# diegoroyo/mitransient

Measured on AMD Instinct MI355X. Metric: Mray/s (closest-hit + shadow rays), Cornell-box 512^2 x 1024 bins x 1024 spp per GPU, higher is better.
Workload: dtype f32; 1 GPU; cornell_box() diffuse, 512x512 px, 1024 time bins (start_opl 3.5, width 6/1024), 1024 spp per GPU (1024 spp total), max_depth 8, rr_depth 5, seed 0; parallelism=1 GPU, mode=auto (fused: scene + per-pixel time histograms in LDS)

## Files before the change

### mitransient_amd/csrc/mtr_core.h

```cpp
#pragma once
#ifndef MTR_WIDE
#define MTR_WIDE 8
#endif

#include <stdint.h>
#include <math.h>
#include "../../include/mitransient_amd.h"

#if defined(__HIPCC__)
#include <hip/hip_runtime.h>
#define MTR_HD __host__ __device__ __forceinline__
#else
#define MTR_HD inline __attribute__((always_inline))
#endif

namespace mtr {

struct f3 { float x, y, z; };

MTR_HD f3 mk(float x, float y, float z) { f3 r; r.x = x; r.y = y; r.z = z; return r; }
MTR_HD f3 operator-(f3 a, f3 b) { return mk(a.x - b.x, a.y - b.y, a.z - b.z); }
MTR_HD f3 operator-(f3 a) { return mk(-a.x, -a.y, -a.z); }
MTR_HD f3 operator*(f3 a, float s) { return mk(a.x * s, a.y * s, a.z * s); }
MTR_HD f3 operator/(f3 a, float s) { float r = 1.0f / s; return mk(a.x * r, a.y * r, a.z * r); }
MTR_HD float dot(f3 a, f3 b) { return fmaf(a.x, b.x, fmaf(a.y, b.y, a.z * b.z)); }
MTR_HD f3 cross(f3 a, f3 b)
{
    return mk(fmaf(a.y, b.z, -(a.z * b.y)), fmaf(a.z, b.x, -(a.x * b.z)), fmaf(a.x, b.y, -(a.y * b.x)));
}
MTR_HD f3 normalize(f3 a) { return a / sqrtf(dot(a, a)); }
MTR_HD f3 fma3(f3 a, float s, f3 b) { return mk(fmaf(a.x, s, b.x), fmaf(a.y, s, b.y), fmaf(a.z, s, b.z)); }
MTR_HD float max3(float a, float b, float c) { return fmaxf(a, fmaxf(b, c)); }
MTR_HD bool sign_neg(float s) { return s < 0.0f || (s == 0.0f && signbit(s)); }

constexpr float kPi = 3.14159265358979323846f;
constexpr float kInvPi = 0.31830988618379067154f;
constexpr float kRayEps = 1500.0f * 5.9604644775390625e-8f;
constexpr float kShadowEps = kRayEps * 10.0f;
constexpr float kInf = __builtin_huge_valf();
constexpr float kEdgeEps = 1.9073486328125e-06f;
// ... 425 lines not shown
        const q4 X = n.q[0], Y = n.q[1], Z = n.q[2], C = n.q[3];
        const bool sx = id.x < 0.0f, sy = id.y < 0.0f, sz = id.z < 0.0f;
        nx = fma2<kPkNodes>(sx ? f2{ X.z, X.w } : f2{ X.x, X.y }, id.x, noid.x); fx = fma2<kPkNodes>(sx ? f2{ X.x, X.y } : f2{ X.z, X.w }, id.x, noid.x);
        ny = fma2<kPkNodes>(sy ? f2{ Y.z, Y.w } : f2{ Y.x, Y.y }, id.y, noid.y); fy = fma2<kPkNodes>(sy ? f2{ Y.x, Y.y } : f2{ Y.z, Y.w }, id.y, noid.y);
        nz = fma2<kPkNodes>(sz ? f2{ Z.z, Z.w } : f2{ Z.x, Z.y }, id.z, noid.z); fz = fma2<kPkNodes>(sz ? f2{ Z.x, Z.y } : f2{ Z.z, Z.w }, id.z, noid.z);
        c0 = (int32_t)fbits(C.x); c1 = (int32_t)fbits(C.y);
    }
    const float tn0 = fmaxf(fmaxf(nx.x, ny.x), fmaxf(nz.x, 0.0f));
    const float tf0 = fminf(fminf(fx.x, fy.x), fminf(fz.x, tb));
    const float tn1 = fmaxf(fmaxf(nx.y, ny.y), fmaxf(nz.y, 0.0f));
    const float tf1 = fminf(fminf(fx.y, fy.y), fminf(fz.y, tb));
    const bool h0 = tn0 <= tf0, h1 = tn1 <= tf1;
    const bool near0 = tn0 <= tn1;
    const bool both = h0 && h1;
    st.push_if(both, near0 ? c1 : c0);
    int32_t nxt = both ? (near0 ? c0 : c1) : (h0 ? c0 : c1);
    if (!(h0 || h1)) nxt = st.empty() ? kTravDone : st.pop();
    tr.cur = nxt;
}

MTR_HD bool is_quad_leaf(int32_t cur) { return cur < 0 && cur != kTravDone && ((~(uint32_t)cur) & kLeafQuadBit) != 0u; }
struct RayOfTrav {
    MTR_HD f3 o(const Trav &tr) const { return tr.o; }
    MTR_HD f3 d(const Trav &tr) const { return tr.d; }
    MTR_HD float tmax(const Trav &tr) const { return tr.tmax; }
};
struct RayByValue {
    f3 ro, rd;
    float rtmax;
    MTR_HD f3 o(const Trav &) const { return ro; }
    MTR_HD f3 d(const Trav &) const { return rd; }
    MTR_HD float tmax(const Trav &) const { return rtmax; }
};
template <class RaySrc = RayOfTrav, class Stack>
MTR_HD bool trav_quad_test(Trav &tr, const SceneView &sc, Stack &st, bool any_hit, const RaySrc ray = RaySrc())
{
    st.count(1);
    const uint32_t first = ((~(uint32_t)tr.cur) & ~kLeafQuadBit) >> 2;
    const TriPair &tp = sc.tpairs[first >> 1];
    const q4 Z = tp.g[0], X = tp.g[1], Y = tp.g[2];
    const uint32_t orig = fbits(tp.g[4].z);
    const f3 o = ray.o(tr), d = ray.d(tr);
    const float oz = fmaf(Z.z, o.z, fmaf(Z.y, o.y, fmaf(Z.x, o.x, Z.w))), dz = fmaf(Z.z, d.z, fmaf(Z.y, d.y, Z.x * d.x));
    const float t = -oz / dz;
    const float ox = fmaf(X.z, o.z, fmaf(X.y, o.y, fmaf(X.x, o.x, X.w))), dx = fmaf(X.z, d.z, fmaf(X.y, d.y, X.x * d.x));
    const float oy = fmaf(Y.z, o.z, fmaf(Y.y, o.y, fmaf(Y.x, o.x, Y.w))), dy = fmaf(Y.z, d.z, fmaf(Y.y, d.y, Y.x * d.x));
    const float lx = fmaf(dx, t, ox), ly = fmaf(dy, t, oy);
    const bool hit = (t >= 0.0f) && (t <= ray.tmax(tr)) && (fabsf(lx) <= 1.0f) && (fabsf(ly) <= 1.0f);
    const bool closer = (t < tr.h.t) | ((t == tr.h.t) & (orig < tr.best_orig));
    const bool better = hit && (any_hit || closer);
    tr.h.t = better ? t : tr.h.t; tr.h.u = better ? lx : tr.h.u; tr.h.v = better ? ly : tr.h.v;
    tr.h.prim = better ? (int32_t)first : tr.h.prim; tr.best_orig = better ? orig : tr.best_orig;
    return hit;
}

template <class RaySrc = RayOfTrav, class Stack>
MTR_HD bool trav_sphere_test(Trav &tr, const SceneView &sc, Stack &st, bool any_hit, const RaySrc ray = RaySrc())
{
    st.count(1);
    const uint32_t first = ((~(uint32_t)tr.cur) & ~kLeafSphereBit) >> 2;
    const TriPair &tp = sc.tpairs[first >> 1];
    const q4 S = tp.g[0];
    const uint32_t orig = fbits(tp.g[4].z);
    const f3 o = ray.o(tr), d = ray.d(tr);
    const f3 l = mk(S.x - o.x, S.y - o.y, S.z - o.z);
    const float tc = dot(l, d);
    const f3 q = mk(fmaf(-d.x, tc, l.x), fmaf(-d.y, tc, l.y), fmaf(-d.z, tc, l.z));
    const float disc = fmaf(S.w, S.w, -dot(q, q));
    const float sq = sqrtf(disc > 0.0f ? disc : 0.0f);
    const float near_t = tc - sq, far_t = tc + sq, maxt = ray.tmax(tr);
    const bool in_bounds = (disc >= 0.0f) && (near_t <= maxt) && (far_t >= 0.0f) && !((near_t < 0.0f) && (far_t > maxt));
    const float t = near_t < 0.0f ? far_t : near_t;
    const bool hit = in_bounds;
    const bool closer = (t < tr.h.t) | ((t == tr.h.t) & (orig < tr.best_orig));
    const bool better = hit && (any_hit || closer);
    if (better) {
        const float k = t - tc;
        const f3 n = normalize(mk(fmaf(d.x, k, -q.x), fmaf(d.y, k, -q.y), fmaf(d.z, k, -q.z)));
        tr.h.t = t; sphere_dir_encode(n, tr.h.u, tr.h.v);
        tr.h.prim = (int32_t)first; tr.best_orig = orig;
    }
    return hit;
}

template <bool ONE_PAIR = false, bool SPH = !ONE_PAIR, class RaySrc = RayOfTrav, class Stack>
MTR_HD bool trav_leaf_test(Trav &tr, const SceneView &sc, Stack &st, bool any_hit, const RaySrc ray = RaySrc())
{
    const uint32_t code = ~(uint32_t)tr.cur;
    if (code & kLeafQuadBit) return trav_quad_test(tr, sc, st, any_hit, ray);
    if constexpr (SPH) { if (code & kLeafSphereBit) return trav_sphere_test(tr, sc, st, any_hit, ray); }
    const uint32_t first = code >> 2, cnt = ONE_PAIR ? (code & 1u) + 1u : (code & 3u) + 1u;
    bool found = false;
    for (uint32_t i = 0; i < (ONE_PAIR ? 1u : cnt); i += 2u) {
        st.count(1);
        const bool two = (i + 1u) < cnt;
        const int32_t pa = (int32_t)(first + i), pb = pa + 1;
        const TriPair &tp = sc.tpairs[(first + i) >> 1];
        const q4 g0 = tp.g[0], g1 = tp.g[1], g2 = tp.g[2], g3 = tp.g[3], g4 = tp.g[4];
        const f2 p0x{ g0.x, g0.y }, p0y{ g0.z, g0.w }, p0z{ g1.x, g1.y };
        const f2 e1x{ g1.z, g1.w }, e1y{ g2.x, g2.y }, e1z{ g2.z, g2.w };
        const f2 e2x{ g3.x, g3.y }, e2y{ g3.z, g3.w }, e2z{ g4.x, g4.y };
        const uint32_t orig_a = fbits(g4.z), orig_b = fbits(g4.w);
        const f3 o = ray.o(tr), d = ray.d(tr);
        const f2 pvx = fma2<kPkLeaf>(e2z, d.y, neg2(mul2<kPkLeaf>(e2y, d.z))), pvy = fma2<kPkLeaf>(e2x, d.z, neg2(mul2<kPkLeaf>(e2z, d.x))), pvz = fma2<kPkLeaf>(e2y, d.x, neg2(mul2<kPkLeaf>(e2x, d.y)));
        const f2 det = fma2<kPkLeaf>(e1x, pvx, fma2<kPkLeaf>(e1y, pvy, mul2<kPkLeaf>(e1z, pvz)));
        const f2 inv_det{ 1.0f / det.x, 1.0f / det.y };
        const f2 tvx = rsub2<kPkLeaf>(o.x, p0x), tvy = rsub2<kPkLeaf>(o.y, p0y), tvz = rsub2<kPkLeaf>(o.z, p0z);
        const f2 u = mul2<kPkLeaf>(fma2<kPkLeaf>(tvx, pvx, fma2<kPkLeaf>(tvy, pvy, mul2<kPkLeaf>(tvz, pvz))), inv_det);
        const f2 qx = fma2<kPkLeaf>(tvy, e1z, neg2(mul2<kPkLeaf>(tvz, e1y))), qy = fma2<kPkLeaf>(tvz, e1x, neg2(mul2<kPkLeaf>(tvx, e1z))), qz = fma2<kPkLeaf>(tvx, e1y, neg2(mul2<kPkLeaf>(tvy, e1x)));
        const f2 v = mul2<kPkLeaf>(fma2<kPkLeaf>(qx, d.x, fma2<kPkLeaf>(qy, d.y, mul2<kPkLeaf>(qz, d.z))), inv_det);
        const f2 t = mul2<kPkLeaf>(fma2<kPkLeaf>(e2x, qx, fma2<kPkLeaf>(e2y, qy, mul2<kPkLeaf>(e2z, qz))), inv_det);
        const f2 w = rsub2<kPkLeaf>(1.0f, add2<kPkLeaf>(u, v));
        {
            const bool hit = (u.x >= -kEdgeEps) && (v.x >= -kEdgeEps) && (w.x >= -kEdgeEps) && (t.x >= 0.0f) && (t.x <= ray.tmax(tr));
            const bool closer = (t.x < tr.h.t) | ((t.x == tr.h.t) & (orig_a < tr.best_orig));
            const bool better = hit && (any_hit ? !found : closer);
            found = found || hit;
            tr.h.t = better ? t.x : tr.h.t; tr.h.u = better ? u.x : tr.h.u; tr.h.v = better ? v.x : tr.h.v;
            tr.h.prim = better ? pa : tr.h.prim; tr.best_orig = better ? orig_a : tr.best_orig;
        }
        {
            const bool hit = two && (u.y >= -kEdgeEps) && (v.y >= -kEdgeEps) && (w.y >= -kEdgeEps) && (t.y >= 0.0f) && (t.y <= ray.tmax(tr));
            const bool closer = (t.y < tr.h.t) | ((t.y == tr.h.t) & (orig_b < tr.best_orig));
            const bool better = hit && (any_hit ? !found : closer);
            found = found || hit;
            tr.h.t = better ? t.y : tr.h.t; tr.h.u = better ? u.y : tr.h.u; tr.h.v = better ? v.y : tr.h.v;
            tr.h.prim = better ? pb : tr.h.prim; tr.best_orig = better ? orig_b : tr.best_orig;
        }
    }
    return found;
// ... 294 lines not shown
    while (tr.cur != kTravDone) {
        const bool at_prim = tr.cur < 0;
        if (__ballot(at_prim) != 0ull) {
            if (is_quad_leaf(tr.cur)) {
                const bool found = trav_quad_test(tr, sc, st, ANY_HIT);
                if (ANY_HIT & found) tr.cur = kTravDone;
                else wide_advance<kWide>(tr, sc.wnodes, st, tr.grp);
            } else if (at_prim) wide_leaf_step<kWide, ONE_PAIR, SPH>(tr, sc, sc.wnodes, st, ANY_HIT);
        } else {
            wide_node_step<kWide, true>(tr, sc.wnodes, st);
        }
    }
#endif
}
#endif

#if defined(__HIPCC__)
template <class T, bool ONE_BASE = false>
__device__ __forceinline__ T kernarg_copy(size_t offset)
{
    static_assert(sizeof(T) % 4 == 0, "dword-sized fields");
    typedef const uint32_t __attribute__((address_space(4))) *WordPtr;
    typedef const char __attribute__((address_space(4))) *BytePtr;
    BytePtr base = (BytePtr)__builtin_amdgcn_kernarg_segment_ptr();
    if (ONE_BASE) asm volatile("" : "+s"(base));
    WordPtr w = (WordPtr)(base + offset);
    if (!ONE_BASE) asm volatile("" : "+s"(w));
    T out;
    uint32_t *o = (uint32_t *)&out;
#pragma unroll
    for (size_t k = 0; k < sizeof(T) / 4; ++k) o[k] = w[k];
    return out;
}
#ifndef MTR_BATCH
#define MTR_BATCH 3
#endif
template <size_t N>
__device__ __forceinline__ void kernarg_pin_words(const uint32_t *o)
{
#define MTR_PIN_W(k) "s"(o[(k) < N ? (k) : N - 1])
    asm volatile("" :: MTR_PIN_W(0), MTR_PIN_W(1), MTR_PIN_W(2), MTR_PIN_W(3), MTR_PIN_W(4), MTR_PIN_W(5), MTR_PIN_W(6), MTR_PIN_W(7),
                       MTR_PIN_W(8), MTR_PIN_W(9), MTR_PIN_W(10), MTR_PIN_W(11), MTR_PIN_W(12), MTR_PIN_W(13), MTR_PIN_W(14), MTR_PIN_W(15));
#undef MTR_PIN_W
    if constexpr (N > 16) kernarg_pin_words<N - 16>(o + 16);
}
template <class T>
__device__ __forceinline__ void kernarg_pin(const T &v)
{
    static_assert(sizeof(T) % 4 == 0, "dword-sized fields");
    kernarg_pin_words<sizeof(T) / 4>((const uint32_t *)&v);
}
#endif

template <class S, class = void> struct stack_one_kernarg_base { static constexpr bool value = false; };
template <class S> struct stack_one_kernarg_base<S, decltype((void)S::kOneKernargBase)> { static constexpr bool value = S::kOneKernargBase; };

#if defined(__HIP_DEVICE_COMPILE__)
template <bool ANY_HIT, uint32_t J, bool BATCH = false>
__device__ __forceinline__ void flat_slab_pair(const f3 id, const f3 noid, const float tb, const uint32_t sel0, const uint32_t sel1, const uint32_t sel2,
                                               const char *root, const bool p0, const bool p1, uint32_t &qm, uint32_t &key1, uint32_t &key2)
{
    const char *pb = root + 48u * J;
    f2 nx, fx, ny, fy, nz, fz;
    if constexpr (BATCH) {
        const f2 pnx = *(const f2 *)(pb + sel0), pfx = *(const f2 *)(pb + (sel0 ^ 8u));
        const f2 pny = *(const f2 *)(pb + sel1), pfy = *(const f2 *)(pb + (sel1 ^ 8u));
        const f2 pnz = *(const f2 *)(pb + sel2), pfz = *(const f2 *)(pb + (sel2 ^ 8u));
        nx = fma2<kPkSlabs>(pnx, id.x, noid.x); fx = fma2<kPkSlabs>(pfx, id.x, noid.x);
        ny = fma2<kPkSlabs>(pny, id.y, noid.y); fy = fma2<kPkSlabs>(pfy, id.y, noid.y);
        nz = fma2<kPkSlabs>(pnz, id.z, noid.z); fz = fma2<kPkSlabs>(pfz, id.z, noid.z);
    } else {
        nx = fma2<kPkSlabs>(*(const f2 *)(pb + sel0), id.x, noid.x); fx = fma2<kPkSlabs>(*(const f2 *)(pb + (sel0 ^ 8u)), id.x, noid.x);
        ny = fma2<kPkSlabs>(*(const f2 *)(pb + sel1), id.y, noid.y); fy = fma2<kPkSlabs>(*(const f2 *)(pb + (sel1 ^ 8u)), id.y, noid.y);
        nz = fma2<kPkSlabs>(*(const f2 *)(pb + sel2), id.z, noid.z); fz = fma2<kPkSlabs>(*(const f2 *)(pb + (sel2 ^ 8u)), id.z, noid.z);
    }
    const float tn0 = fmaxf(fmaxf(nx.x, ny.x), fmaxf(nz.x, 0.0f));
    const float tf0 = fminf(fminf(fx.x, fy.x), fminf(fz.x, tb));
    const float tn1 = fmaxf(fmaxf(nx.y, ny.y), fmaxf(nz.y, 0.0f));
    const float tf1 = fminf(fminf(fx.y, fy.y), fminf(fz.y, tb));
    const bool h0 = (tn0 <= tf0) && p0;
    const bool h1 = (tn1 <= tf1) && p1;
    qm |= (h0 ? 1u : 0u) << (2u * J);
    qm |= (h1 ? 2u : 0u) << (2u * J);
    if (!ANY_HIT) {
        const uint32_t ka = h0 ? ((fbits(tn0) & ~7u) | (2u * J)) : 0xffffffffu, kb = h1 ? ((fbits(tn1) & ~7u) | (2u * J + 1u)) : 0xffffffffu;
        key2 = min(key2, max(key1, ka)); key1 = min(key1, ka);
        key2 = min(key2, max(key1, kb)); key1 = min(key1, kb);
    }
}
template <bool ANY_HIT, bool ONE_PAIR, bool TOP_LEAVES, class Stack>
__device__ __forceinline__ Hit flat_walk_device(const SceneView &sc, const f3 o, const f3 d, const float tmax, Stack &st)
{
    typedef WNode N;
    Trav tr;
    const RayByValue ray{ o, d, tmax };
    tr.h.t = kInf; tr.h.u = 0.0f; tr.h.v = 0.0f; tr.h.prim = -1;
    tr.best_orig = 0xffffffffu;
    st.reset();
    if (!sc.n_slots) return tr.h;
    const char *root = (const char *)sc.wnodes;
    constexpr bool kOneBase = stack_one_kernarg_base<Stack>::value;
    const FlatHdr fh = kernarg_copy<FlatHdr, kOneBase>(sc.flat_off);
    bool live = true;
    uint32_t fm = 0u;
    const float omax = fmaxf(fmaxf(fabsf(o.x), fabsf(o.y)), fabsf(o.z));
    for (uint32_t b = 0; b < fh.n_boxes; ++b) {
        const FlatXf X = kernarg_copy<FlatXf, kOneBase>(sc.flat_off + sizeof(FlatHdr) + sizeof(FlatXf) * b);
        const q4 A = X.A, B = X.B, C = X.C, S = X.S;
        const f3 ol = mk(fmaf(A.z, o.z, fmaf(A.y, o.y, fmaf(A.x, o.x, A.w))), fmaf(B.z, o.z, fmaf(B.y, o.y, fmaf(B.x, o.x, B.w))),
                         fmaf(C.z, o.z, fmaf(C.y, o.y, fmaf(C.x, o.x, C.w))));
        const f3 dl = mk(fmaf(A.z, d.z, fmaf(A.y, d.y, A.x * d.x)), fmaf(B.z, d.z, fmaf(B.y, d.y, B.x * d.x)),
                         fmaf(C.z, d.z, fmaf(C.y, d.y, C.x * d.x)));
        const f3 id = mk(safe_rcp(dl.x), safe_rcp(dl.y), safe_rcp(dl.z));
        fm |= box_select(box_mag_bound(A, B, C, S, omax), ol, dl, id, tmax) << (6u * b);
    }
    st.prof_flat(0);
    while (__ballot(live && fm != 0u) != 0ull) {
        if (live && fm != 0u) {
            const uint32_t k = (uint32_t)__builtin_ctz(fm);
            fm &= fm - 1u;
            const uint32_t box = (k * 43u) >> 8, face = k - 6u * box;
            tr.cur = *(const int32_t *)(root + (size_t)(fh.node0 + box) * N::kBytes + N::kRefOff + 4u * face);
            const bool found = trav_leaf_test<true>(tr, sc, st, ANY_HIT, ray);
            if (ANY_HIT && found) live = false;
        }
    }
    st.prof_flat(5);
    if (__ballot(live) != 0ull) {
        const f3 id = mk(safe_rcp(d.x), safe_rcp(d.y), safe_rcp(d.z));
        const f3 noid = mk(-(o.x * id.x), -(o.y * id.y), -(o.z * id.z));
        const uint32_t sel0 = id.x < 0.0f ? 8u : 0u, sel1 = 16u + (id.y < 0.0f ? 8u : 0u), sel2 = 32u + (id.z < 0.0f ? 8u : 0u);
        const float tb = fminf(tmax, tr.h.t);
        uint32_t qm = 0u;
        uint32_t key1 = 0xffffffffu, key2 = 0xffffffffu;
#define MTR_FLAT_SLAB_PAIR(J) flat_slab_pair<ANY_HIT, J, kOneBase && (MTR_BATCH & 1) != 0>(id, noid, tb, sel0, sel1, sel2, root, \
            TOP_LEAVES ? ((fh.prim_mask >> (2u * J)) & 1u) != 0u : 2u * J < fh.n_quads, \
            TOP_LEAVES ? ((fh.prim_mask >> (2u * J + 1u)) & 1u) != 0u : 2u * J + 1u < fh.n_quads, qm, key1, key2)
        if (TOP_LEAVES) {
            MTR_FLAT_SLAB_PAIR(0u);
            if (fh.prim_mask > 3u) MTR_FLAT_SLAB_PAIR(1u);
            if (fh.prim_mask > 15u) MTR_FLAT_SLAB_PAIR(2u);
            if (kWide > 6u && fh.prim_mask > 63u) MTR_FLAT_SLAB_PAIR(3u);
        } else {
            MTR_FLAT_SLAB_PAIR(0u); MTR_FLAT_SLAB_PAIR(1u); MTR_FLAT_SLAB_PAIR(2u);
            if (kWide > 6u && fh.n_quads > 6u) MTR_FLAT_SLAB_PAIR(3u);
        }
#undef MTR_FLAT_SLAB_PAIR
        if (!live) qm = 0u;
        st.prof_flat(2);
        for (uint32_t it = 0; __ballot(qm != 0u) != 0ull; ++it) {
            if (qm != 0u) {
                const uint32_t k = (!ANY_HIT && it == 0u) ? (key1 & 7u) : (uint32_t)__builtin_ctz(qm);
                qm &= ~(1u << k);
                tr.cur = *(const int32_t *)(root + N::kRefOff + 4u * k);
                const bool found = (!TOP_LEAVES || is_quad_leaf(tr.cur)) ? trav_quad_test(tr, sc, st, ANY_HIT, ray)
                                                                         : trav_leaf_test<ONE_PAIR, false>(tr, sc, st, ANY_HIT, ray);
                if (ANY_HIT ? found : (it == 0u && tr.h.t < bitsf(key2 & ~7u))) qm = 0u;
            }
        }
    }
    st.prof_flat(4);
    return tr.h;
}
#endif

template <bool ANY_HIT, bool ONE_PAIR = false, int FLAT = 0, bool SPH = !ONE_PAIR && FLAT == 0, class Stack>
MTR_HD Hit traverse(const SceneView &sc, f3 o, f3 d, float tmax, Stack &st)
{
#if defined(__HIP_DEVICE_COMPILE__)
    if (FLAT) return flat_walk_device<ANY_HIT, ONE_PAIR, FLAT == 2>(sc, o, d, tmax, st);
#endif
    Trav tr;
    trav_init(tr, sc, o, d, tmax, st);
#ifdef MTR_PROFILE_SIMT
    uint32_t my_nodes = 0;
#endif
    if (sc.wnodes) {
#if defined(__HIP_DEVICE_COMPILE__) && !defined(MTR_NODES_FIRST)
        wide_walk_device<ANY_HIT, ONE_PAIR, SPH>(tr, sc, st);
#else
        while (tr.cur != kTravDone) {
            while (tr.cur >= 0) {
                wide_node_step<kWide, true>(tr, sc.wnodes, st);
#ifdef MTR_PROFILE_SIMT
                ++my_nodes;
#endif
            }
            if (is_quad_leaf(tr.cur)) {
                const bool found = trav_quad_test(tr, sc, st, ANY_HIT);
                if (ANY_HIT & found) tr.cur = kTravDone;
// ... 960 lines not shown
    if (!kDiff) p.eta *= bs.eta;
    p.beta = mk(p.beta.x * bs.w.x, p.beta.y * bs.w.y, p.beta.z * bs.w.z);
    p.prev_p = sp; p.prev_pdf = bs.pdf;
    if (!kDiff) p.prev_delta = bs.delta ? 1u : 0u;

    float bmax = max3(p.beta.x, p.beta.y, p.beta.z);
    active_next &= (bmax != 0.0f);
    float rr_prob = fminf(kDiff ? bmax : bmax * (p.eta * p.eta), 0.95f);
    active_next &= rr_prob > 0.0f;
    bool rr_active = p.depth >= rc.rr_depth;
    if (rr_active) {
        float inv = rr_prob > 0.0f ? 1.0f / rr_prob : 0.0f;
        p.beta = p.beta * inv;
    }
    active_next &= (!rr_active) | (rr_u < rr_prob);
    if (valid) p.depth += 1;
    return active_next;
}

struct NoRefresh { template <class Sink> MTR_HD void operator()(Path &, Sink &) const {} };
template <bool ROUGH = true, uint32_t TR = 0u, class Stack, class Sink, class Refresh = NoRefresh>
MTR_HD bool path_bounce(Path &p, const SceneView &sc, const Film &film, const RenderConst &rc,
                        Stack &st, Sink &sink, BounceStats &stats, const Refresh &refresh = Refresh(), bool unwarp_here = false)
{
    st.prof_mark(2);
    Hit h = traverse<false, (TR & kTrLeafPair) != 0u, flat_kind(TR), tr_spheres(TR)>(sc, p.ray.o, p.ray.d, p.ray.tmax, st);
    st.prof_mark(0);
    stats.closest++;
    Pending pd; Ray shadow;
    shadow.o = mk(0, 0, 0); shadow.d = mk(0, 0, 1); shadow.tmax = 0.0f;
    if (Stack::kPark) { p.prev_p = st.unpark_prev_p(); p.prev_pdf = st.unpark_prev_pdf(); p.rng.inc = st.unpark_inc(); }
    refresh(p, sink);
    if (unwarp_here && p.depth == 0u && h.prim >= 0) p.dist = -h.t;
    shade_hit<ROUGH, TR>(p, h, sc, film, rc, sink, pd, shadow);
    st.prof_mark(1);
    bool occluded = false;
    if (pd.has_shadow) {
        stats.shadow++;
        Hit sh = traverse<true, (TR & kTrLeafPair) != 0u, flat_kind(TR), tr_spheres(TR)>(sc, shadow.o, shadow.d, shadow.tmax, st);
        occluded = sh.prim >= 0;
    }
    st.prof_mark(0);
    if (Stack::kPark) p.rng.inc = st.unpark_inc();
    refresh(p, sink);
    const bool an = shade_finish<ROUGH, TR>(p, h, occluded, pd, sc, film, rc, sink);
    if (Stack::kPark) { st.park_prev_p(p.prev_p); st.park_prev_pdf(p.prev_pdf); }
    st.prof_mark(1);
    return an;
}

template <class Sink>
MTR_HD void commit_pending(f3 &L, f3 Lr, float opl, uint32_t depth_log, uint32_t px, uint32_t py,
                           const Film &film, const RenderConst &rc, Sink &sink)
{
    const uint32_t fx = px - film.crop_x, fy = py - film.crop_y;
    const float vr = Lr.x * rc.sample_scale, vg = Lr.y * rc.sample_scale, vb = Lr.z * rc.sample_scale;
    if ((fx < film.width) & (fy < film.height) && (vr != 0.0f || vg != 0.0f || vb != 0.0f)) {
        const int32_t bin = film_bin(film, opl);
        if (bin >= 0) sink.splat(fx, fy, (uint32_t)bin, vr, vg, vb, opl, depth_log, 1u);
    }
    L = mk(L.x + Lr.x, L.y + Lr.y, L.z + Lr.z);
}

}
```

### mitransient_amd/csrc/mtr_kernels.hip

```cpp
#include "mtr_kernels.h"
#include "mtr_knobs.h"

#include <hip/hip_runtime.h>
#include <algorithm>
#include <type_traits>
#include <hip/amd_detail/amd_hip_unsafe_atomics.h>

namespace mtr {

template <bool ONE_BASE = false>
struct LdsStackT {
    static constexpr bool kOneKernargBase = ONE_BASE;
    int32_t *base;
    int sp;
    __device__ __forceinline__ void reset() { sp = 0; }
    __device__ __forceinline__ void push_if(bool c, int32_t v) { base[sp * kBlock] = v; sp += c ? 1 : 0; }
    __device__ __forceinline__ int32_t pop() { --sp; return base[sp * kBlock]; }
    __device__ __forceinline__ bool empty() const { return sp == 0; }
#ifndef MTR_NO_PARK
    static constexpr bool kPark = true;
    static constexpr uint32_t kParkRows = 6;
    int park_row;
    __device__ __forceinline__ void park_prev_p(f3 v) { base[(park_row + 0) * kBlock] = (int32_t)fbits(v.x); base[(park_row + 1) * kBlock] = (int32_t)fbits(v.y); base[(park_row + 2) * kBlock] = (int32_t)fbits(v.z); }
    __device__ __forceinline__ f3 unpark_prev_p() const { return mk(bitsf((uint32_t)base[(park_row + 0) * kBlock]), bitsf((uint32_t)base[(park_row + 1) * kBlock]), bitsf((uint32_t)base[(park_row + 2) * kBlock])); }
// ... 169 lines not shown
    uint32_t n_splats;
    SplatLog log;
    __device__ __forceinline__ void splat(uint32_t fx, uint32_t fy, uint32_t bin, float r, float g, float b,
                                          float opl, uint32_t depth, uint32_t kind)
    {
        size_t idx = (((size_t)fy * film_w + fx) * bins + bin) * 4u;
        unsafeAtomicAdd(film + idx, r); unsafeAtomicAdd(film + idx + 1, g); unsafeAtomicAdd(film + idx + 2, b);
        ++n_splats;
        if (log.rec) log_splat(log, lane, depth, kind, fy * film_w + fx, bin, r, g, b, opl);
    }
};

__device__ __forceinline__ void copy16(void *dst, const void *src, uint32_t bytes, int tid)
{
    const uint4 *s = (const uint4 *)src; uint4 *d = (uint4 *)dst;
    for (uint32_t i = tid; i < bytes / 16u; i += kBlock) d[i] = s[i];
}
__host__ __device__ constexpr uint32_t align16(uint32_t x) { return (x + 15u) & ~15u; }

struct LoopArgs { uint32_t spp_begin, spp_chunk, G; FastDiv div_spp, div_G; };
static_assert(offsetof(FusedArgs, spp_chunk) - offsetof(FusedArgs, spp_begin) == offsetof(LoopArgs, spp_chunk) &&
              offsetof(FusedArgs, G) - offsetof(FusedArgs, spp_begin) == offsetof(LoopArgs, G) &&
              offsetof(FusedArgs, div_spp) - offsetof(FusedArgs, spp_begin) == offsetof(LoopArgs, div_spp) &&
              offsetof(FusedArgs, div_G) - offsetof(FusedArgs, spp_begin) == offsetof(LoopArgs, div_G), "LoopArgs mirrors FusedArgs");
#ifndef MTR_FUSED_MIN_WAVES
#define MTR_FUSED_MIN_WAVES 4
#endif
template <bool SCENE_LDS, bool HIST_LDS, bool NLOS, int MINW = MTR_FUSED_MIN_WAVES, bool PHASOR = false, bool FIXED = false, bool ROUGH = false, uint32_t TR = 0u>
__global__ void __launch_bounds__(kBlock, MINW) k_fused(const FusedArgs a)
{
    extern __shared__ __attribute__((aligned(16))) unsigned char smem[];
    const int tid = threadIdx.x;
    constexpr bool kLean = SCENE_LDS && HIST_LDS && !NLOS && !PHASOR && !FIXED && !ROUGH && flat_kind(TR) != 0;
#ifdef MTR_PROFILE_TAIL
    const unsigned long long t0_wall = wall_clock64();
#endif

    uint32_t off = 0;
    int32_t *s_stack = (int32_t *)(smem + off); off += (a.stack_rows + (NLOS ? 0u : LdsStack::kParkRows)) * kBlock * 4;
    unsigned long long *s_cnt = (unsigned long long *)(smem + off); off += 64;
    uint32_t *s_next = (uint32_t *)(s_cnt + 6);
    SceneView sv;
    sv.n_emitters = a.sc.n_ems; sv.n_slots = a.sc.n_slots;
    sv.samp_tris = a.sc.samp_tris; sv.samp_vn = a.sc.samp_vn; sv.face_pmf = a.sc.face_pmf; sv.face_cdf = a.sc.face_cdf; sv.vnormals = a.sc.vnormals;
    sv.texels = a.sc.texels; sv.tex_info = a.sc.tex_info; sv.uvs = a.sc.uvs;
    sv.flat_off = (uint32_t)(offsetof(FusedArgs, sc) + offsetof(SceneDev, flat));
    if (SCENE_LDS) {
        const uint32_t tree_bytes = a.sc.n_wnodes * (uint32_t)sizeof(WNode);
        WNode *n = (WNode *)(smem + off); off += align16(tree_bytes);
        TriPair *tg = (TriPair *)(smem + off); off += align16(a.sc.n_slots / 2 * sizeof(TriPair));
        TriShade *ts = (TriShade *)(smem + off); off += align16(a.sc.n_slots * sizeof(TriShade));
        mtr_material *mm = (mtr_material *)(smem + off); off += align16(a.sc.n_mats * sizeof(mtr_material));
        Emitter *ee = (Emitter *)(smem + off); off += align16(a.sc.n_ems * sizeof(Emitter));
        copy16(n, a.sc.wnodes, align16(tree_bytes), tid);
        copy16(tg, a.sc.tpairs, align16(a.sc.n_slots / 2 * sizeof(TriPair)), tid);
        copy16(ts, a.sc.tshade, align16(a.sc.n_slots * sizeof(TriShade)), tid);
        copy16(mm, a.sc.mats, align16(a.sc.n_mats * sizeof(mtr_material)), tid);
        copy16(ee, a.sc.ems, align16(a.sc.n_ems * sizeof(Emitter)), tid);
        sv.nodes = nullptr; sv.wnodes = n; sv.wnodes4 = nullptr; sv.wnodes8q = nullptr; sv.tpairs = tg; sv.tshade = ts; sv.mats = mm; sv.ems = ee;
        sv.node_pairs = true;
        __builtin_assume(sv.wnodes != nullptr);
    } else {
        sv.nodes = a.sc.nodes; sv.tpairs = a.sc.tpairs; sv.tshade = a.sc.tshade; sv.mats = a.sc.mats; sv.ems = a.sc.ems;
        sv.wnodes = nullptr; sv.wnodes4 = a.sc.wnodes4; sv.wnodes8q = a.sc.wnodes8q;
        sv.node_pairs = false;
    }
    const uint32_t K = a.G;
    float *s_steady = (float *)(smem + off); off += align16(K * 32);
    unsigned long long *s_steady64 = (unsigned long long *)s_steady;
    float *s_steady_ovf = (float *)(smem + off); if (FIXED) off += align16(K * 16);
    uint32_t *s_owner = (uint32_t *)(smem + off); off += align16(K * 4);
    uint32_t *s_done = (uint32_t *)(smem + off); off += align16(K * 4);
    float *s_hist = (float *)(smem + off);
    const uint32_t T = PHASOR ? 2u * a.film.n_freq : a.film.bins;
    constexpr bool kGrey = (TR & kTrGrey) != 0u;
    const uint32_t plane = kGrey ? 0u : K * T;

    if (tid < 6) s_cnt[tid] = 0ull;
    for (uint32_t k = tid; k < K; k += kBlock) s_done[k] = 0u;
    for (uint32_t k = tid; k < K * 8; k += kBlock) s_steady[k] = 0.0f;
    unsigned long long *s_hist64 = (unsigned long long *)s_hist;
// ... 351 lines not shown
    }
#endif
#ifdef MTR_PROFILE_CYCLES
    if ((tid & 63) == 0 && a.counters) {
        st.prof_mark(5);
        unsigned long long *c = &a.counters->splats_overflow;
#if MTR_PROFILE_CYCLES == 3
        atomicAdd(c + 0, st.cyc[0]); atomicAdd(c + 1, st.cyc[1]); atomicAdd(c + 2, (st.cyc[3] << 32) | ((st.cyc[2] >> 6) & 0xffffffffull));
#else
        atomicAdd(c + 0, ((st.cyc[0] >> 10) << 32) | (st.cyc[1] >> 10));
        atomicAdd(c + 1, ((st.cyc[2] >> 10) << 32) | (st.cyc[3] >> 10));
        atomicAdd(c + 2, ((st.cyc[4] >> 10) << 32) | (st.cyc[5] >> 10));
#endif
    }
#endif
}

static uint32_t scene_lds_bytes(const SceneDev &sc)
{
    return align16(sc.n_wnodes * sizeof(WNode)) + align16(sc.n_slots / 2 * sizeof(TriPair)) +
           align16(sc.n_slots * sizeof(TriShade)) + align16(sc.n_mats * sizeof(mtr_material)) +
           align16(sc.n_ems * sizeof(Emitter));
}

uint32_t fused_chunk(uint32_t n_pixels, uint32_t spp_chunk, uint32_t grid)
{
    uint32_t chunk = (32768u + spp_chunk - 1u) / (spp_chunk ? spp_chunk : 1u);
    const uint32_t c_bal = (uint32_t)((unsigned long long)n_pixels / (2ull * (unsigned long long)(grid ? grid : 1u)));
    if (chunk > c_bal) chunk = c_bal;
    if (chunk < 1u) chunk = 1u;
    return fused_chunk_cap(chunk, spp_chunk);
}

bool fused_plan(const SceneDev &sc, const Film &film, uint32_t n_pixels, uint32_t spp_chunk, int n_cu,
                FusedArgs &args, FusedConfig &cfg)
{
    const uint32_t kLdsMax = 160u * 1024u;
    int stack = sc.bvh_depth <= 8 ? 8 : sc.bvh_depth <= 16 ? 16 : sc.bvh_depth <= 32 ? 32 : 64;
    if (sc.bvh_depth > 64) return false;
    if ((uint64_t)film.crop_x + film.crop_w > 65536ull || (uint64_t)film.crop_y + film.crop_h > 65536ull) return false;
    uint32_t scene_b = scene_lds_bytes(sc);
    cfg.scene_lds = sc.wnodes != nullptr && scene_b <= 64u * 1024u;
    const uint32_t rows = wf_stack_rows(sc, cfg.scene_lds);
    args.stack_rows = rows;
    uint32_t fixed_b = (rows + (args.nlos_on ? 0u : LdsStack::kParkRows)) * kBlock * 4 + 64;
    if (cfg.scene_lds) fixed_b += scene_b;
    const bool det = (args.rc.flags & MTR_FLAG_DETERMINISTIC) && !film.n_freq;
    cfg.rough = sc.has_rough != 0u;
    const bool grey = args.nlos_on && !film.n_freq && !det && cfg.scene_lds && (sc.traits & kTrGrey) && (!cfg.rough || (sc.traits & kTrNoLobes)) &&
                      film.bins * 4u <= 48u * 1024u && !mtr::knob("MTR_NO_GREY");
    const uint32_t row_bytes = film.n_freq ? film.n_freq * 8u : film.bins * (det ? 36u : grey ? 4u : 12u);
    cfg.fixed = false;
    const uint32_t hist_budget = (det ? 108u : 48u) * 1024u;
    args.fixed_dcap = args.rc.max_depth < 64u ? (args.rc.max_depth ? args.rc.max_depth : 1u) : 64u;
    args.fixed_lim = 1048576.0f / (2.0f * (float)(spp_chunk ? spp_chunk : 1u) * (float)args.fixed_dcap);
    uint32_t g_want = (MTR_FUSED_SEG_LANES + spp_chunk - 1u) / (spp_chunk ? spp_chunk : 1u);
    if (g_want < 1) g_want = 1;
    uint32_t g_fit = row_bytes ? hist_budget / row_bytes : 1u;
    cfg.hist_lds = true;
    uint32_t G;
    if (g_fit >= 1) G = g_want < g_fit ? g_want : g_fit;
    else if (fixed_b + row_bytes + 64 <= kLdsMax) G = 1;
    else { G = g_want; cfg.hist_lds = false; }
    if (film.n_freq && !cfg.hist_lds) return false;
    cfg.fixed = det && cfg.hist_lds;
    cfg.traits = (cfg.rough ? (sc.traits & kTrNoLobes) : (sc.traits & ~kTrNoLobes)) & ~kTrGrey;
    if (grey) cfg.traits |= kTrGrey;
    if (!args.nlos_on && !film.n_freq && !cfg.rough && cfg.scene_lds && cfg.hist_lds &&
        (cfg.fixed ? cfg.traits == kTrCornellFlat : (cfg.traits & kTrFlatFlags) == kTrFlatFlags)) {
        fixed_b -= rows * kBlock * 4;
        args.stack_rows = 0u;
    }
    const int reg_cap = (cfg.rough || cfg.fixed || args.nlos_on) ? 3 : (int)MTR_FUSED_MIN_WAVES;
    auto lds_of = [&](uint32_t g) { return (size_t)fixed_b + align16(g * 32) + (cfg.fixed ? align16(g * 16) : 0u) + 2 * align16(g * 4) + (cfg.hist_lds ? (size_t)g * row_bytes : 0) + 16; };
    auto per_cu_of = [&](uint32_t g) { const int p = (int)(kLdsMax / lds_of(g)); return p > reg_cap ? reg_cap : p; };
    if (cfg.hist_lds) {
        uint32_t best = G;
        for (uint32_t g = G; g-- > 1u;) if (per_cu_of(g) > per_cu_of(best)) best = g;
        G = best;
    }
    if (const char *e = mtr::knob("MTR_FUSED_G")) { const uint32_t v = (uint32_t)atoi(e); if (v >= 1u && v < G && cfg.hist_lds) G = v; }
    if (G > n_pixels) G = n_pixels ? n_pixels : 1;
    if (G > 4096) G = 4096;
    args.G = G;
    args.div_G = fastdiv_make(G); args.div_spp = fastdiv_make(spp_chunk);
    cfg.stack = stack;
    cfg.lds_bytes = lds_of(G);
    if (cfg.lds_bytes > kLdsMax) return false;
    int per_cu = per_cu_of(G);
    if (per_cu < 1) per_cu = 1;
    if (const char *e = mtr::knob("MTR_FUSED_PER_CU")) { const int v = atoi(e); if (v >= 1 && v < per_cu) per_cu = v; }
    if (mtr::knob("MTR_FUSED_VERBOSE")) fprintf(stderr, "fused_plan: G %u, row %u B, lds %zu B, per_cu %d, traits %u, rough %d, fixed %d\n", G, row_bytes, (size_t)cfg.lds_bytes, per_cu, cfg.traits, (int)cfg.rough, (int)cfg.fixed);
    cfg.per_cu = per_cu;
    long grid = (long)n_cu * per_cu;
    uint32_t g_blk = g_want;
    while (g_blk > 1 && ((long)n_pixels + g_blk - 1) / g_blk < n_cu && (unsigned long long)g_blk * spp_chunk > 512ull) g_blk = (g_blk + 1) / 2;
    const long max_blocks = ((long)n_pixels + g_blk - 1) / g_blk;
    if (grid > max_blocks) grid = max_blocks;
    if (grid < 1) grid = 1;
    uint32_t chunk = fused_chunk(n_pixels, spp_chunk, (uint32_t)grid);
    if (const char *e = mtr::knob("MTR_FUSED_CHUNK")) { const int v = atoi(e); if (v >= 1) chunk = fused_chunk_cap((uint32_t)v, spp_chunk); }
    if ((unsigned long long)chunk * spp_chunk > 0xffff0000ull) return false;
    args.chunk = chunk;
    args.n_chunks = (n_pixels + chunk - 1u) / chunk;
    if (grid > (long)args.n_chunks) grid = args.n_chunks;
    cfg.grid = (int)grid;
    return true;
}

#ifndef MTR_C2_TRAITS
#define MTR_C2_TRAITS kTrCornellFlat
#endif
template <bool NLOS>
static hipError_t launch_fused_s(const FusedArgs &args, const FusedConfig &cfg, hipStream_t stream)
{
    void (*k)(const FusedArgs) = nullptr;
#ifdef MTR_ONLY_C2
    if (NLOS || args.film.n_freq || cfg.rough || cfg.fixed || !cfg.scene_lds || !cfg.hist_lds || cfg.traits != MTR_C2_TRAITS || cfg.per_cu <= 3) return hipErrorInvalidValue;
    k = k_fused<true, true, false, MTR_FUSED_MIN_WAVES, false, false, false, MTR_C2_TRAITS>;
#else
    if (args.film.n_freq) {
        if (!cfg.hist_lds || cfg.rough) return hipErrorInvalidValue;
        if constexpr (NLOS) k = cfg.scene_lds ? k_fused<true, true, true, 3, true> : k_fused<false, true, true, 3, true>;
        else k = cfg.scene_lds ? k_fused<true, true, false, MTR_FUSED_MIN_WAVES, true> : k_fused<false, true, false, MTR_FUSED_MIN_WAVES, true>;
    }
    else if (cfg.rough) {
        if (cfg.fixed) return hipErrorInvalidValue;
        if (NLOS && (cfg.traits & kTrGrey)) { if constexpr (NLOS) k = k_fused<true, true, true, 3, false, false, true, kTrNoLobes | kTrGrey>; }
        else if (cfg.scene_lds && cfg.hist_lds && (cfg.traits & kTrNoLobes)) k = k_fused<true, true, NLOS, 3, false, false, true, kTrNoLobes>;
        else
        k = cfg.scene_lds ? (cfg.hist_lds ? k_fused<true, true, NLOS, 3, false, false, true> : k_fused<true, false, NLOS, 3, false, false, true>)
                          : (cfg.hist_lds ? k_fused<false, true, NLOS, 3, false, false, true> : k_fused<false, false, NLOS, 3, false, false, true>);
    }
    else if (cfg.fixed) {
        k = cfg.scene_lds ? k_fused<true, true, NLOS, 3, false, true> : k_fused<false, true, NLOS, 3, false, true>;
        if constexpr (!NLOS) if (cfg.scene_lds && cfg.traits == kTrCornellFlat) k = k_fused<true, true, false, 3, false, true, false, kTrCornellFlat>;
    }
    else if (!NLOS && cfg.scene_lds && cfg.hist_lds && cfg.traits == kTrCornellFlat)
        k = cfg.per_cu <= 3 ? k_fused<true, true, false, 3, false, false, false, kTrCornellFlat> : k_fused<true, true, false, MTR_FUSED_MIN_WAVES, false, false, false, kTrCornellFlat>;
    else if (!NLOS && cfg.scene_lds && cfg.hist_lds && (cfg.traits & kTrFlatGeneral) == kTrFlatFlags)
        k = cfg.per_cu <= 3 ? k_fused<true, true, false, 3, false, false, false, kTrFlatFlags> : k_fused<true, true, false, MTR_FUSED_MIN_WAVES, false, false, false, kTrFlatFlags>;
    else if (!NLOS && cfg.scene_lds && cfg.hist_lds && (cfg.traits & kTrFlatGeneral) == kTrFlatGeneral)
        k = cfg.per_cu <= 3 ? k_fused<true, true, false, 3, false, false, false, kTrFlatGeneral> : k_fused<true, true, false, MTR_FUSED_MIN_WAVES, false, false, false, kTrFlatGeneral>;
    else if (!NLOS && cfg.scene_lds && cfg.hist_lds && (cfg.traits & kTrCornell) == kTrCornell)
        k = cfg.per_cu <= 3 ? k_fused<true, true, false, 3, false, false, false, kTrCornell> : k_fused<true, true, false, MTR_FUSED_MIN_WAVES, false, false, false, kTrCornell>;
    else if (NLOS && (cfg.traits & kTrGrey)) {
        if constexpr (NLOS) k = k_fused<true, true, true, 3, false, false, false, kTrGrey>;
    }
    else if (cfg.scene_lds && cfg.hist_lds) {
        if constexpr (NLOS) k = k_fused<true, true, true, 3>;
        else k = cfg.per_cu <= 3 ? k_fused<true, true, false, 3> : k_fused<true, true, false>;
    }
    else if (cfg.scene_lds && !cfg.hist_lds) k = k_fused<true, false, NLOS>;
    else if (!cfg.scene_lds && cfg.hist_lds) k = k_fused<false, true, NLOS>;
    else k = k_fused<false, false, NLOS>;
#endif
    hipError_t e = hipFuncSetAttribute((const void *)k, hipFuncAttributeMaxDynamicSharedMemorySize, (int)cfg.lds_bytes);
    if (e != hipSuccess) return e;
    e = hipMemsetAsync(args.ticket, 0, sizeof(uint32_t), stream);
    if (e != hipSuccess) return e;
    hipLaunchKernelGGL(k, dim3(cfg.grid), dim3(kBlock), cfg.lds_bytes, stream, args);
    return hipGetLastError();
}

__global__ void __launch_bounds__(kBlock) k_nlos_prepare(SceneDev sc, NlosConst nc, q4 *targets)
{
    extern __shared__ __attribute__((aligned(16))) unsigned char smem[];
    LdsStack st; st.base = (int32_t *)smem + threadIdx.x; st.sp = 0;
    SceneView sv;
    sv.nodes = sc.nodes; sv.tpairs = sc.tpairs; sv.tshade = sc.tshade; sv.mats = sc.mats; sv.ems = sc.ems;
    sv.wnodes = nullptr; sv.wnodes4 = nullptr; sv.wnodes8q = nullptr;
    sv.node_pairs = false;
    sv.n_emitters = sc.n_ems; sv.n_slots = sc.n_slots;
    sv.samp_tris = sc.samp_tris; sv.samp_vn = sc.samp_vn; sv.face_pmf = sc.face_pmf; sv.face_cdf = sc.face_cdf; sv.vnormals = sc.vnormals;
// ... 283 lines not shown
```

Before: 41290 Mray/s.

## Stage flat-scene primitive records in a compact LDS table and hand over hit context

Adds an LDS-resident table holding the flat scene's top-level quads and box faces as contiguous TriPair records with their prim indices. The lean flat walk then fetches records straight from this table rather than reading a node reference and following it through the tpairs array, which removes a dependent load per leaf test. It also changes the default MTR_BATCH from 3 to 15, which turns on this table and a new path that passes the hit context from shade_hit to shade_finish for Cornell-style scenes. The cost is extra LDS per block, which may lower how many blocks fit on a CU, plus more template variants.

```diff
diff --git a/mitransient_amd/csrc/mtr_core.h b/mitransient_amd/csrc/mtr_core.h
--- a/mitransient_amd/csrc/mtr_core.h
+++ b/mitransient_amd/csrc/mtr_core.h
@@ -2,10 +2,14 @@
 #ifndef MTR_WIDE
 #define MTR_WIDE 8
 #endif
+#ifndef MTR_BATCH
+#define MTR_BATCH 15
+#endif
 
 #include <stdint.h>
 #include <math.h>
 #include "../../include/mitransient_amd.h"
+#include "mtr_flat_prims.h"
 
 #if defined(__HIPCC__)
 #include <hip/hip_runtime.h>
@@ -497,12 +501,26 @@
     MTR_HD f3 d(const Trav &) const { return rd; }
     MTR_HD float tmax(const Trav &) const { return rtmax; }
 };
-template <class RaySrc = RayOfTrav, class Stack>
-MTR_HD bool trav_quad_test(Trav &tr, const SceneView &sc, Stack &st, bool any_hit, const RaySrc ray = RaySrc())
+struct RecOfLeaf {
+    static constexpr bool kPairsOnly = false;
+    MTR_HD uint32_t quad_first(const Trav &tr) const { return ((~(uint32_t)tr.cur) & ~kLeafQuadBit) >> 2; }
+    MTR_HD uint32_t leaf_code(const Trav &tr) const { return ~(uint32_t)tr.cur; }
+    MTR_HD const TriPair &pair(const SceneView &sc, uint32_t slot) const { return sc.tpairs[slot >> 1]; }
+};
+struct RecByValue {
+    static constexpr bool kPairsOnly = true;
+    TriPair tp;
+    uint32_t first;
+    MTR_HD uint32_t quad_first(const Trav &) const { return first; }
+    MTR_HD uint32_t leaf_code(const Trav &) const { return (first << 2) | 1u; }
+    MTR_HD const TriPair &pair(const SceneView &, uint32_t) const { return tp; }
+};
+template <class RaySrc = RayOfTrav, class RecSrc = RecOfLeaf, class Stack>
+MTR_HD bool trav_quad_test(Trav &tr, const SceneView &sc, Stack &st, bool any_hit, const RaySrc ray = RaySrc(), const RecSrc rec = RecSrc())
 {
     st.count(1);
-    const uint32_t first = ((~(uint32_t)tr.cur) & ~kLeafQuadBit) >> 2;
-    const TriPair &tp = sc.tpairs[first >> 1];
+    const uint32_t first = rec.quad_first(tr);
+    const TriPair &tp = rec.pair(sc, first);
     const q4 Z = tp.g[0], X = tp.g[1], Y = tp.g[2];
     const uint32_t orig = fbits(tp.g[4].z);
     const f3 o = ray.o(tr), d = ray.d(tr);
@@ -548,19 +566,21 @@
     return hit;
 }
 
-template <bool ONE_PAIR = false, bool SPH = !ONE_PAIR, class RaySrc = RayOfTrav, class Stack>
-MTR_HD bool trav_leaf_test(Trav &tr, const SceneView &sc, Stack &st, bool any_hit, const RaySrc ray = RaySrc())
-{
-    const uint32_t code = ~(uint32_t)tr.cur;
-    if (code & kLeafQuadBit) return trav_quad_test(tr, sc, st, any_hit, ray);
-    if constexpr (SPH) { if (code & kLeafSphereBit) return trav_sphere_test(tr, sc, st, any_hit, ray); }
+template <bool ONE_PAIR = false, bool SPH = !ONE_PAIR, class RaySrc = RayOfTrav, class RecSrc = RecOfLeaf, class Stack>
+MTR_HD bool trav_leaf_test(Trav &tr, const SceneView &sc, Stack &st, bool any_hit, const RaySrc ray = RaySrc(), const RecSrc rec = RecSrc())
+{
+    const uint32_t code = rec.leaf_code(tr);
+    if constexpr (!RecSrc::kPairsOnly) {
+        if (code & kLeafQuadBit) return trav_quad_test(tr, sc, st, any_hit, ray);
+        if constexpr (SPH) { if (code & kLeafSphereBit) return trav_sphere_test(tr, sc, st, any_hit, ray); }
+    }
     const uint32_t first = code >> 2, cnt = ONE_PAIR ? (code & 1u) + 1u : (code & 3u) + 1u;
     bool found = false;
     for (uint32_t i = 0; i < (ONE_PAIR ? 1u : cnt); i += 2u) {
         st.count(1);
         const bool two = (i + 1u) < cnt;
         const int32_t pa = (int32_t)(first + i), pb = pa + 1;
-        const TriPair &tp = sc.tpairs[(first + i) >> 1];
+        const TriPair &tp = rec.pair(sc, first + i);
         const q4 g0 = tp.g[0], g1 = tp.g[1], g2 = tp.g[2], g3 = tp.g[3], g4 = tp.g[4];
         const f2 p0x{ g0.x, g0.y }, p0y{ g0.z, g0.w }, p0z{ g1.x, g1.y };
         const f2 e1x{ g1.z, g1.w }, e1y{ g2.x, g2.y }, e1z{ g2.z, g2.w };
@@ -921,9 +941,7 @@
     for (size_t k = 0; k < sizeof(T) / 4; ++k) o[k] = w[k];
     return out;
 }
-#ifndef MTR_BATCH
-#define MTR_BATCH 3
-#endif
+constexpr bool flat_prim_table_on(bool lean, bool top_leaves) { return lean && !top_leaves && (MTR_BATCH & 4) != 0 && kWide <= kFlatPrimQuads; }
 template <size_t N>
 __device__ __forceinline__ void kernarg_pin_words(const uint32_t *o)
 {
@@ -977,6 +995,15 @@
         key2 = min(key2, max(key1, kb)); key1 = min(key1, kb);
     }
 }
+__device__ __forceinline__ RecByValue flat_prim_fetch(const char *root, const uint32_t n_boxes, const uint32_t entry)
+{
+    const char *tab = root - flat_prim_bytes(n_boxes);
+    const TriPair *p = (const TriPair *)(tab + flat_prim_rec_off(entry));
+    RecByValue r;
+    r.tp.g[0] = p->g[0]; r.tp.g[1] = p->g[1]; r.tp.g[2] = p->g[2]; r.tp.g[3] = p->g[3]; r.tp.g[4] = p->g[4];
+    r.first = *(const uint32_t *)(tab + flat_prim_first_off(n_boxes, entry));
+    return r;
+}
 template <bool ANY_HIT, bool ONE_PAIR, bool TOP_LEAVES, class Stack>
 __device__ __forceinline__ Hit flat_walk_device(const SceneView &sc, const f3 o, const f3 d, const float tmax, Stack &st)
 {
@@ -989,7 +1016,8 @@
     if (!sc.n_slots) return tr.h;
     const char *root = (const char *)sc.wnodes;
     constexpr bool kOneBase = stack_one_kernarg_base<Stack>::value;
-    const FlatHdr fh = kernarg_copy<FlatHdr, kOneBase>(sc.flat_off);
+    constexpr bool kTable = flat_prim_table_on(kOneBase, TOP_LEAVES);
+    const FlatHdr fh =kernarg_copy<FlatHdr, kOneBase>(sc.flat_off);
     bool live = true;
     uint32_t fm = 0u;
     const float omax = fmaxf(fmaxf(fabsf(o.x), fabsf(o.y)), fabsf(o.z));
@@ -1008,10 +1036,16 @@
         if (live && fm != 0u) {
             const uint32_t k = (uint32_t)__builtin_ctz(fm);
             fm &= fm - 1u;
-            const uint32_t box = (k * 43u) >> 8, face = k - 6u * box;
-            tr.cur = *(const int32_t *)(root + (size_t)(fh.node0 + box) * N::kBytes + N::kRefOff + 4u * face);
-            const bool found = trav_leaf_test<true>(tr, sc, st, ANY_HIT, ray);
-            if (ANY_HIT && found) live = false;
+            if constexpr (kTable) {
+                const RecByValue rec = flat_prim_fetch(root, fh.n_boxes, kFlatPrimQuads + k);
+                const bool found = trav_leaf_test<true, false>(tr, sc, st, ANY_HIT, ray, rec);
+                if (ANY_HIT && found) live = false;
+            } else {
+                const uint32_t box = (k * 43u) >> 8, face = k - 6u * box;
+                tr.cur = *(const int32_t *)(root + (size_t)(fh.node0 + box) * N::kBytes + N::kRefOff + 4u * face);
+                const bool found = trav_leaf_test<true>(tr, sc, st, ANY_HIT, ray);
+                if (ANY_HIT && found) live = false;
+            }
         }
     }
     st.prof_flat(5);
@@ -1041,10 +1075,16 @@
             if (qm != 0u) {
                 const uint32_t k = (!ANY_HIT && it == 0u) ? (key1 & 7u) : (uint32_t)__builtin_ctz(qm);
                 qm &= ~(1u << k);
-                tr.cur = *(const int32_t *)(root + N::kRefOff + 4u * k);
-                const bool found = (!TOP_LEAVES || is_quad_leaf(tr.cur)) ? trav_quad_test(tr, sc, st, ANY_HIT, ray)
-                                                                         : trav_leaf_test<ONE_PAIR, false>(tr, sc, st, ANY_HIT, ray);
-                if (ANY_HIT ? found : (it == 0u && tr.h.t < bitsf(key2 & ~7u))) qm = 0u;
+                if constexpr (kTable) {
+                    const RecByValue rec = flat_prim_fetch(root, fh.n_boxes, flat_prim_quad_entry(k));
+                    const bool found = trav_quad_test(tr, sc, st, ANY_HIT, ray, rec);
+                    if (ANY_HIT ? found : (it == 0u && tr.h.t < bitsf(key2 & ~7u))) qm = 0u;
+                } else {
+                    tr.cur = *(const int32_t *)(root + N::kRefOff + 4u * k);
+                    const bool found = (!TOP_LEAVES || is_quad_leaf(tr.cur)) ? trav_quad_test(tr, sc, st, ANY_HIT, ray)
+                                                                             : trav_leaf_test<ONE_PAIR, false>(tr, sc, st, ANY_HIT, ray);
+                    if (ANY_HIT ? found : (it == 0u && tr.h.t < bitsf(key2 & ~7u))) qm = 0u;
+                }
             }
         }
     }
@@ -2071,7 +2111,9 @@
     if (Stack::kPark) { p.prev_p = st.unpark_prev_p(); p.prev_pdf = st.unpark_prev_pdf(); p.rng.inc = st.unpark_inc(); }
     refresh(p, sink);
     if (unwarp_here && p.depth == 0u && h.prim >= 0) p.dist = -h.t;
-    shade_hit<ROUGH, TR>(p, h, sc, film, rc, sink, pd, shadow);
+    constexpr bool kHandOver = stack_one_kernarg_base<Stack>::value && flat_kind(TR) == 1 && (TR & kTrCornell) == kTrCornell && (MTR_BATCH & 8) != 0;
+    HitCtx kept;
+    shade_hit<ROUGH, TR>(p, h, sc, film, rc, sink, pd, shadow, kHandOver ? &kept : nullptr);
     st.prof_mark(1);
     bool occluded = false;
     if (pd.has_shadow) {
@@ -2082,7 +2124,7 @@
     st.prof_mark(0);
     if (Stack::kPark) p.rng.inc = st.unpark_inc();
     refresh(p, sink);
-    const bool an = shade_finish<ROUGH, TR>(p, h, occluded, pd, sc, film, rc, sink);
+    const bool an = shade_finish<ROUGH, TR>(p, h, occluded, pd, sc, film, rc, sink, kHandOver ? &kept : nullptr);
     if (Stack::kPark) { st.park_prev_p(p.prev_p); st.park_prev_pdf(p.prev_pdf); }
     st.prof_mark(1);
     return an;
diff --git a/mitransient_amd/csrc/mtr_flat_prims.h b/mitransient_amd/csrc/mtr_flat_prims.h
--- /dev/null
+++ b/mitransient_amd/csrc/mtr_flat_prims.h
@@ -0,0 +1,24 @@
+#pragma once
+#include <cstdint>
+
+#if defined(__HIPCC__)
+#define MTR_FP_HD __host__ __device__ constexpr
+#else
+#define MTR_FP_HD constexpr
+#endif
+
+namespace mtr {
+
+constexpr uint32_t kFlatPrimQuads = 8;
+constexpr uint32_t kFlatPrimFaces = 6;
+constexpr uint32_t kFlatPrimRecBytes = 80;
+constexpr uint32_t kFlatPrimEntryBytes = kFlatPrimRecBytes + 4u;
+
+MTR_FP_HD uint32_t flat_prim_entries(uint32_t n_boxes) { return kFlatPrimQuads + kFlatPrimFaces * n_boxes; }
+MTR_FP_HD uint32_t flat_prim_quad_entry(uint32_t k) { return k; }
+MTR_FP_HD uint32_t flat_prim_face_entry(uint32_t b, uint32_t f) { return kFlatPrimQuads + kFlatPrimFaces * b + f; }
+MTR_FP_HD uint32_t flat_prim_rec_off(uint32_t entry) { return kFlatPrimRecBytes * entry; }
+MTR_FP_HD uint32_t flat_prim_first_off(uint32_t n_boxes, uint32_t entry) { return kFlatPrimRecBytes * flat_prim_entries(n_boxes) + 4u * entry; }
+MTR_FP_HD uint32_t flat_prim_bytes(uint32_t n_boxes) { return (kFlatPrimEntryBytes * flat_prim_entries(n_boxes) + 15u) & ~15u; }
+
+}
diff --git a/mitransient_amd/csrc/mtr_kernels.hip b/mitransient_amd/csrc/mtr_kernels.hip
--- a/mitransient_amd/csrc/mtr_kernels.hip
+++ b/mitransient_amd/csrc/mtr_kernels.hip
@@ -225,6 +225,7 @@
     extern __shared__ __attribute__((aligned(16))) unsigned char smem[];
     const int tid = threadIdx.x;
     constexpr bool kLean = SCENE_LDS && HIST_LDS && !NLOS && !PHASOR && !FIXED && !ROUGH && flat_kind(TR) != 0;
+    constexpr bool kPrimTable = flat_prim_table_on(kLean, flat_kind(TR) == 2);
 #ifdef MTR_PROFILE_TAIL
     const unsigned long long t0_wall = wall_clock64();
 #endif
@@ -240,6 +241,25 @@
     sv.flat_off = (uint32_t)(offsetof(FusedArgs, sc) + offsetof(SceneDev, flat));
     if (SCENE_LDS) {
         const uint32_t tree_bytes = a.sc.n_wnodes * (uint32_t)sizeof(WNode);
+        if constexpr (kPrimTable) {
+            static_assert(sizeof(TriPair) == kFlatPrimRecBytes && kFlatMaxBoxes * kFlatPrimFaces + kFlatPrimQuads <= 32u, "mtr_flat_prims.h");
+            const uint32_t nb = a.sc.flat.n_boxes, n_ent = flat_prim_entries(nb);
+            unsigned char *tab = smem + off; off += flat_prim_bytes(nb);
+            constexpr uint32_t kWords = kFlatPrimEntryBytes / 4u;
+            for (uint32_t w = tid; w < n_ent * kWords; w += kBlock) {
+                const uint32_t e = w / kWords, j = w - kWords * e;
+                const bool quad = e < kFlatPrimQuads;
+                const uint32_t b = quad ? 0u : (e - kFlatPrimQuads) / kFlatPrimFaces, f = quad ? e : (e - kFlatPrimQuads) - kFlatPrimFaces * b;
+                const uint32_t node = quad ? 0u : a.sc.flat.node0 + b;
+                uint32_t v = 0u;
+                if ((!quad || e < a.sc.flat.n_quads) && node < a.sc.n_wnodes) {
+                    const uint32_t code = ~(uint32_t)a.sc.wnodes[node].ref[f];
+                    const uint32_t first = (quad ? code & ~kLeafQuadBit : code) >> 2;
+                    if (first < a.sc.n_slots) v = j < kWords - 1u ? ((const uint32_t *)(a.sc.tpairs + (first >> 1)))[j] : first;
+                }
+                *(uint32_t *)(tab + (j < kWords - 1u ? flat_prim_rec_off(e) + 4u * j : flat_prim_first_off(nb, e))) = v;
+            }
+        }
         WNode *n = (WNode *)(smem + off); off += align16(tree_bytes);
         TriPair *tg = (TriPair *)(smem + off); off += align16(a.sc.n_slots / 2 * sizeof(TriPair));
         TriShade *ts = (TriShade *)(smem + off); off += align16(a.sc.n_slots * sizeof(TriShade));
@@ -657,6 +677,15 @@
     return fused_chunk_cap(chunk, spp_chunk);
 }
 
+static bool fused_lean_flat_quads(bool nlos_on, uint32_t n_freq, const FusedConfig &cfg)
+{
+    return !nlos_on && !n_freq && !cfg.rough && !cfg.fixed && cfg.scene_lds && cfg.hist_lds && (cfg.traits & kTrFlatGeneral) == kTrFlatFlags;
+}
+static uint32_t fused_prim_table_bytes(const SceneDev &sc, bool nlos_on, uint32_t n_freq, const FusedConfig &cfg)
+{
+    return flat_prim_table_on(true, false) && fused_lean_flat_quads(nlos_on, n_freq, cfg) ? flat_prim_bytes(sc.flat.n_boxes) : 0u;
+}
+
 bool fused_plan(const SceneDev &sc, const Film &film, uint32_t n_pixels, uint32_t spp_chunk, int n_cu,
                 FusedArgs &args, FusedConfig &cfg)
 {
@@ -696,6 +725,7 @@
         fixed_b -= rows * kBlock * 4;
         args.stack_rows = 0u;
     }
+    fixed_b += fused_prim_table_bytes(sc, args.nlos_on != 0u, film.n_freq, cfg);
     const int reg_cap = (cfg.rough || cfg.fixed || args.nlos_on) ? 3 : (int)MTR_FUSED_MIN_WAVES;
     auto lds_of = [&](uint32_t g) { return (size_t)fixed_b + align16(g * 32) + (cfg.fixed ? align16(g * 16) : 0u) + 2 * align16(g * 4) + (cfg.hist_lds ? (size_t)g * row_bytes : 0) + 16; };
     auto per_cu_of = [&](uint32_t g) { const int p = (int)(kLdsMax / lds_of(g)); return p > reg_cap ? reg_cap : p; };
@@ -761,10 +791,14 @@
         k = cfg.scene_lds ? k_fused<true, true, NLOS, 3, false, true> : k_fused<false, true, NLOS, 3, false, true>;
         if constexpr (!NLOS) if (cfg.scene_lds && cfg.traits == kTrCornellFlat) k = k_fused<true, true, false, 3, false, true, false, kTrCornellFlat>;
     }
-    else if (!NLOS && cfg.scene_lds && cfg.hist_lds && cfg.traits == kTrCornellFlat)
-        k = cfg.per_cu <= 3 ? k_fused<true, true, false, 3, false, false, false, kTrCornellFlat> : k_fused<true, true, false, MTR_FUSED_MIN_WAVES, false, false, false, kTrCornellFlat>;
-    else if (!NLOS && cfg.scene_lds && cfg.hist_lds && (cfg.traits & kTrFlatGeneral) == kTrFlatFlags)
-        k = cfg.per_cu <= 3 ? k_fused<true, true, false, 3, false, false, false, kTrFlatFlags> : k_fused<true, true, false, MTR_FUSED_MIN_WAVES, false, false, false, kTrFlatFlags>;
+    else if (fused_lean_flat_quads(NLOS, 0u, cfg)) {
+        if constexpr (!NLOS) {
+            if (cfg.traits == kTrCornellFlat)
+                k = cfg.per_cu <= 3 ? k_fused<true, true, false, 3, false, false, false, kTrCornellFlat> : k_fused<true, true, false, MTR_FUSED_MIN_WAVES, false, false, false, kTrCornellFlat>;
+            else
+                k = cfg.per_cu <= 3 ? k_fused<true, true, false, 3, false, false, false, kTrFlatFlags> : k_fused<true, true, false, MTR_FUSED_MIN_WAVES, false, false, false, kTrFlatFlags>;
+        }
+    }
     else if (!NLOS && cfg.scene_lds && cfg.hist_lds && (cfg.traits & kTrFlatGeneral) == kTrFlatGeneral)
         k = cfg.per_cu <= 3 ? k_fused<true, true, false, 3, false, false, false, kTrFlatGeneral> : k_fused<true, true, false, MTR_FUSED_MIN_WAVES, false, false, false, kTrFlatGeneral>;
     else if (!NLOS && cfg.scene_lds && cfg.hist_lds && (cfg.traits & kTrCornell) == kTrCornell)
```

New measurement: 42690 Mray/s, median of 6. 3.4% higher.
